# Amanda-Zheng/MR-GNAS

Hardware: AMD Instinct MI355X
Metric: million edges/sec per supernet fwd+bwd step (FB15k-237, dim=200) (higher is better)
Workload: dtype f32

## Files before the change

### mr-gnas_amd/csrc/wgrad.hip

```cpp
#include "x3_parts.hpp"
#include "wgrad_plan.hpp"

static_assert(mrg::WGRAD_BLOCK == MRG_BLOCK, "wgrad_plan.hpp plans for workgroups of MRG_BLOCK threads");

namespace mrg {

struct WgradArgs {
  const float* gY; int Nout; int ldg;
  const float* X1; const float* X2; int K1, K2;
  float* ws;
  int64_t rows, rows_per_block;
  int TM, TN, TNB;
  int ngrp;
  int64_t g_lo[3], g_hi[3], g_rpb[3], g_ws_off[3];
  int g_G[3];
};

struct XSel { const float* base; int ld, kk; };
__device__ __forceinline__ XSel wgrad_sel_x(const WgradArgs& a, int c) {
  const bool first = c < a.K1 || a.K2 == 0;
  XSel s;
  s.base = first ? a.X1 : a.X2;
  s.ld = first ? a.K1 : a.K2;
  s.kk = first ? c : c - a.K1;
// ... 391 lines not shown
  const int tn0 = (int)(((int64_t)blockIdx.y * a.TN) / gridDim.y);
  const int tnb = (int)(((int64_t)(blockIdx.y + 1) * a.TN) / gridDim.y) - tn0;
  const int tid = threadIdx.x, wave = __builtin_amdgcn_readfirstlane(tid >> 6), lane = tid & 63, li = lane & 31, lh = lane >> 5;
  const int wg = wave / KP, wp = wave % KP;
  const int m0 = wg * 4;
  const int an = a.TM - m0 < 4 ? (a.TM - m0 > 0 ? a.TM - m0 : 0) : 4;
  const int kn = tnb - 2 * wp < 2 ? (tnb - 2 * wp > 0 ? tnb - 2 * wp : 0) : 2;
  const int K = a.K1 + a.K2;

  f32x16 acc[4][2];
#pragma unroll
  for (int i = 0; i < 4; ++i)
#pragma unroll
    for (int j = 0; j < 2; ++j)
#pragma unroll
      for (int r = 0; r < 16; ++r) acc[i][j][r] = 0.f;

  int64_t r_begin = (int64_t)blockIdx.x * a.rows_per_block;
  int64_t r_end = r_begin + a.rows_per_block;
  if (r_end > a.rows) r_end = a.rows;
  int64_t ws_off = 0;
  if (a.ngrp > 0) {
    const int z = blockIdx.z;
#define MRG_PICKZ(F) (z == 0 ? a.F[0] : (z == 1 ? a.F[1] : a.F[2]))
    if ((int)blockIdx.x >= MRG_PICKZ(g_G)) return;
    const int64_t rpb = MRG_PICKZ(g_rpb), hi = MRG_PICKZ(g_hi);
    r_begin = MRG_PICKZ(g_lo) + (int64_t)blockIdx.x * rpb;
    r_end = r_begin + rpb < hi ? r_begin + rpb : hi;
    ws_off = MRG_PICKZ(g_ws_off);
#undef MRG_PICKZ
  }

  const float* src[FPW]; int64_t ld[FPW]; bool live[FPW];
#pragma unroll
  for (int i = 0; i < FPW; ++i) {
    const int f = wave + 8 * i;
    live[i] = f < NFRAG && (f < ASLOTS ? f < a.TM : f - ASLOTS < tnb);
    const float* base = mrg_zeros16; int64_t l = 0;
    if (live[i]) {
      if (f < ASLOTS) {
        const int cg = f * 32 + li;
        if (cg < a.Nout) { base = a.gY + (r_begin + 8 * lh) * a.ldg + cg; l = a.ldg; }
      } else {
        const int cg = (tn0 + f - ASLOTS) * 32 + li;
        if (cg < K) {
          const XSel sx = wgrad_sel_x(a, cg);
          base = sx.base + (r_begin + 8 * lh) * sx.ld + sx.kk; l = sx.ld;
        } else if (cg == K) {
          base = mrg_ones16;
        }
      }
    }
    src[i] = base; ld[i] = l;
  }
  constexpr unsigned BUF_BYTES = X::BUF_BYTES;

  const int64_t nfull = (r_end - r_begin) / WBR;
  const int nv_tail = (int)((r_end - r_begin) - nfull * WBR);
  const int kbase = 8 * lh;
  float raw[FPW][8];
  auto fetch = [&](int64_t t) {
    const int64_t toff = t * WBR;
#pragma unroll
    for (int i = 0; i < FPW; ++i) {
      const float* p = src[i] + toff * ld[i];
#pragma unroll
      for (int j = 0; j < 8; ++j) raw[i][j] = p[j * ld[i]];
    }
  };
  auto produce = [&](int buf, auto tail_c) {
    constexpr bool TAIL = decltype(tail_c)::value;
#pragma unroll
    for (int i = 0; i < FPW; ++i) {
      if (live[i]) {
        float x[8];
#pragma unroll
        for (int j = 0; j < 8; ++j) x[j] = (!TAIL || kbase + j < nv_tail) ? raw[i][j] : 0.f;
        u32x4 H, M, L;
        split8(x, H, M, L);
        const int f = wave + 8 * i;
        u32x4* dst = reinterpret_cast<u32x4*>(reinterpret_cast<char*>(smem) + buf * BUF_BYTES + f * X::FRAG_BYTES) + lane;
        dst[0] = H; dst[64] = M; dst[128] = L;
      }
    }
  };
  auto rdfrag = [&](int buf, int f, bf16x8& H, bf16x8& M, bf16x8& L) {
    const u32x4* p = reinterpret_cast<const u32x4*>(reinterpret_cast<const char*>(smem) + buf * BUF_BYTES + f * X::FRAG_BYTES) + lane;
    H = __builtin_bit_cast(bf16x8, p[0]); M = __builtin_bit_cast(bf16x8, p[64]); L = __builtin_bit_cast(bf16x8, p[128]);
  };
  auto consume = [&](int cur) {
    if (an > 0 && kn > 0) {
      bf16x8 Bh0, Bm0, Bl0, Bh1, Bm1, Bl1;
      rdfrag(cur, ASLOTS + 2 * wp, Bh0, Bm0, Bl0);
      if (kn > 1) rdfrag(cur, ASLOTS + 2 * wp + 1, Bh1, Bm1, Bl1);
      else { Bh1 = Bh0; Bm1 = Bm0; Bl1 = Bl0; }
      bf16x8 An[3];
      rdfrag(cur, m0, An[0], An[1], An[2]);
#pragma unroll
      for (int i = 0; i < 4; ++i) {
        if (i < an) {
          const bf16x8 Ah = An[0], Am = An[1], Al = An[2];
          if (i + 1 < an) rdfrag(cur, m0 + i + 1, An[0], An[1], An[2]);
          if (kn > 1) {
            x3_chain2(acc[i][0], acc[i][1], Ah, Am, Al, Bh0, Bm0, Bl0, Ah, Am, Al, Bh1, Bm1, Bl1);
          } else {
            x3_chain(acc[i][0], Ah, Am, Al, Bh0, Bm0, Bl0);
          }
        }
      }
    }
  };

  if (nfull > 0) {
    fetch(0);
    produce(0, std::false_type{});
    fetch(nfull > 1 ? 1 : 0);
    __syncthreads();
    int cur = 0;
    for (int64_t t = 0; t < nfull; ++t) {
      consume(cur);
      if (t + 1 < nfull) produce(cur ^ 1, std::false_type{});
      fetch(t + 2 < nfull ? t + 2 : nfull - 1);
      __syncthreads();
      cur ^= 1;
    }
  }
  if (nv_tail > 0) {
    const int64_t toff = nfull * WBR;
#pragma unroll
    for (int i = 0; i < FPW; ++i) {
      const float* p = src[i] + toff * ld[i];
#pragma unroll
      for (int j = 0; j < 8; ++j) raw[i][j] = p[(int64_t)(kbase + j >= nv_tail ? j - WBR : j) * ld[i]];
    }
    produce(0, std::true_type{});
    __syncthreads();
    consume(0);
  }
  const int ldw = a.TN * 32;
  float* out = a.ws + ws_off + (int64_t)blockIdx.x * (a.TM * 32) * ldw;
#pragma unroll
  for (int i = 0; i < 4; ++i)
#pragma unroll
    for (int j = 0; j < 2; ++j)
      if (i < an && j < kn) {
#pragma unroll
        for (int r = 0; r < 16; ++r) {
          const int row = (m0 + i) * 32 + (r & 3) + 8 * (r >> 2) + 4 * lh;
          out[(int64_t)row * ldw + (tn0 + 2 * wp + j) * 32 + li] = acc[i][j][r];
        }
      }
}

static int launch_wgrad_x3(const WgradArgs& a, int G, int nrange, hipStream_t st) {
  bool v1 = gemm_switches().wgrad_variant == 1 && a.rows >= WBR;
  for (int i = 0; i < a.ngrp; ++i) v1 = v1 && !(a.g_hi[i] > a.g_lo[i] && a.g_hi[i] < WBR);
  auto go = [&](auto ng_c) {
    using X = WgradX3<decltype(ng_c)::value>;
    const dim3 grid(G, (a.TN + X::KT - 1) / X::KT, nrange);
    if (v1) return launch_kernel(wgrad_x3v_k<decltype(ng_c)::value>, grid, dim3(WX_THREADS), X::LDS_SPLIT, st, a);
    return launch_kernel(wgrad_x3_k<decltype(ng_c)::value>, grid, dim3(WX_THREADS), X::LDS_RAW, st, a);
  };
  return a.TM <= 4 ? go(std::integral_constant<int, 1>{}) : go(std::integral_constant<int, 2>{});
}

struct WgradReduce3 { const float* ws[3]; float* gW[3]; float* gbias[3]; int G[3]; };
__global__ void wgrad_reduce3_k(WgradReduce3 p, int K, int Nout, int ldg, int ldx) {
  __shared__ float part[16][64];
  const int z = blockIdx.z;
  const float* __restrict__ ws = z == 0 ? p.ws[0] : (z == 1 ? p.ws[1] : p.ws[2]);
  float* __restrict__ gW = z == 0 ? p.gW[0] : (z == 1 ? p.gW[1] : p.gW[2]);
  float* __restrict__ gbias = z == 0 ? p.gbias[0] : (z == 1 ? p.gbias[1] : p.gbias[2]);
  const int G = z == 0 ? p.G[0] : (z == 1 ? p.G[1] : p.G[2]);
  if (!gW) return;
  const int tx = threadIdx.x & 63, ty = threadIdx.x >> 6;
  const int c = blockIdx.x * 64 + tx;
  const int n = blockIdx.y;
  float acc = 0.f;
  if (c <= K)
    for (int g = ty; g < G; g += 16) acc += ws[((int64_t)g * ldg + n) * ldx + c];
  part[ty][tx] = acc;
  __syncthreads();
  if (ty == 0 && c <= K) {
    float tot = part[0][tx];
#pragma unroll
    for (int i = 1; i < 16; ++i) tot += part[i][tx];
    if (c < K) gW[(int64_t)n * K + c] = tot;
    else if (gbias) gbias[n] = tot;
  }
}

static int launch_wgrad_reduce(const WgradReduce3& red, int nrange, int K, int Nout, int TM, int TN, hipStream_t st) {
  hipLaunchKernelGGL(wgrad_reduce3_k, dim3((K + 1 + 63) / 64, Nout, nrange), dim3(1024), 0, st, red, K, Nout, TM * 32, TN * 32);
  MRG_LAUNCH_CHECK();
  return MRG_OK;
}

static int64_t wgrad_workspace_bytes(int64_t rows, int K, int Nout) {
  WgradPlan p = wgrad_plan(rows, K, Nout);
  return (int64_t)p.G * p.TM * 32 * p.TN * 32 * sizeof(float);
}

static bool wgrad_vec_ok(const float* gY, int ldg, const float* X1, const float* X2, int K1, int K2, int Nout) {
  const bool shape = Nout >= 4 && Nout % 4 == 0 && ldg % 4 == 0 && K1 >= 4 && K1 % 4 == 0 && K2 >= 0 && K2 % 4 == 0;
  return shape && aligned16(gY) && aligned16(X1) && (!X2 || K2 == 0 || aligned16(X2));
}

static int launch_wgrad_one(const float* gY, int ldg, const float* X1, const float* X2, int K1, int K2, float* gW, float* gbias, void* ws,
                            int64_t rows, int Nout, int share, hipStream_t st) {
  const int K = K1 + K2;
  if (rows == 0) {
    hipError_t e = hipMemsetAsync(gW, 0, sizeof(float) * (size_t)Nout * K, st);
    if (e == hipSuccess && gbias) e = hipMemsetAsync(gbias, 0, sizeof(float) * (size_t)Nout, st);
    return (int)e;
  }
  const bool vec = Nout <= 224 && wgrad_vec_ok(gY, ldg, X1, X2, K1, K2, Nout);
  WgradPlan p = wgrad_plan(rows, K, Nout, vec, share);
  if (!p.ok) return MRG_E_SHAPE;
  WgradArgs a{};
  a.gY = gY; a.Nout = Nout; a.ldg = ldg; a.X1 = X1; a.X2 = X2; a.K1 = K1; a.K2 = K2; a.ws = (float*)ws;
  a.rows = rows; a.rows_per_block = p.rows_per_block; a.TM = p.TM; a.TN = p.TN; a.TNB = p.TNB;
  if (!X2 || K2 == 0) { a.X2 = X1; a.K2 = 0; }
  int rc = MRG_E_SHAPE;
  if (vec && gemm_switches().mode != 1) {
    rc = launch_wgrad_x3(a, p.G, 1, st);
  } else {
    const dim3 grid(p.G, (p.TN + p.TNB - 1) / p.TNB);
    const int npf = wgrad_npf_class(p.npf);
    void (*kernel)(WgradArgs) = nullptr;
#define MRG_WGRAD_DMA(T, F) if (vec && p.tpw == T && npf == F) kernel = wgrad_dma_k<T, F>;
#define MRG_WGRAD_PLAIN(T, F) if (!vec && p.tpw == T && npf == F) kernel = wgrad_k<T, F>;
    MRG_WGRAD_DMA_INSTANCES(MRG_WGRAD_DMA) MRG_WGRAD_PLAIN_INSTANCES(MRG_WGRAD_PLAIN)
#undef MRG_WGRAD_DMA
#undef MRG_WGRAD_PLAIN
    if (kernel) rc = launch_kernel(kernel, grid, dim3(MRG_BLOCK), p.lds, st, a);
  }
  if (rc != MRG_OK) return rc;
  const WgradReduce3 red{{(const float*)ws}, {gW}, {gbias}, {p.G}};
  return launch_wgrad_reduce(red, 1, K, Nout, p.TM, p.TN, st);
}

struct Wgrad3Layout { int64_t lo[3], hi[3], off[3], total; WgradPlan plan[3]; };
static Wgrad3Layout wgrad3_layout(int64_t b0, int64_t b1, int64_t M, int K, int Nout, int share) {
  Wgrad3Layout L{{0, b0, b1}, {b0, b1, M}};
  for (int i = 0; i < 3; ++i) {
    L.plan[i] = wgrad_plan(L.hi[i] - L.lo[i], K, Nout, true, share);
    L.off[i] = L.total;
    L.total += (wgrad_workspace_bytes(L.hi[i] - L.lo[i], K, Nout) + 255) / 256 * 256;
  }
  return L;
}

}

using namespace mrg;

extern "C" int mrg_wgrad_set_variant(int variant) {
  if (variant != 0 && variant != 1) return MRG_E_ENUM;
  gemm_switches().wgrad_variant = variant;
  return MRG_OK;
}

extern "C" int64_t mrg_linear_bwd_weight3_workspace_bytes(int64_t b0, int64_t b1, int64_t M, int K1, int K2, int Nout) {
  if (M < 0 || b0 < 0 || b1 < b0 || M < b1 || Nout > 224 || !wgrad_vec_ok(nullptr, Nout, nullptr, nullptr, K1, K2, Nout) || gemm_switches().mode == 1) return 0;
  return wgrad3_layout(b0, b1, M, K1 + K2, Nout, 1).total;
}

extern "C" int mrg_linear_bwd_weight3(const float* gY, const float* X1, const float* X2, float* const* gW_host, float* const* gb_host, void* ws,
                                      int64_t b0, int64_t b1, int64_t M, int K1, int K2, int Nout, void* stream) {
  if (M < 0 || b0 < 0 || b1 < b0 || M < b1 || Nout > 224 || !wgrad_vec_ok(nullptr, Nout, nullptr, nullptr, K1, K2, Nout)) return MRG_E_SHAPE;
  if (!gW_host) return MRG_E_NULLPTR;
  if (M > 0 && (!gY || !X1 || (K2 > 0 && !X2))) return MRG_E_NULLPTR;
  if (!ws) return MRG_E_WORKSPACE;
  if (!wgrad_vec_ok(gY, Nout, X1, X2, K1, K2, Nout)) return MRG_E_SHAPE;
  const int K = K1 + K2;
  const int64_t rows[3] = {b0, b1 - b0, M - b1};
  int nlive = 0;
  for (int i = 0; i < 3; ++i) nlive += (gW_host[i] != nullptr && rows[i] > 0) ? 1 : 0;
  const Wgrad3Layout L = wgrad3_layout(b0, b1, M, K, Nout, nlive < 1 ? 1 : nlive);
  if (!L.plan[0].ok) return MRG_E_SHAPE;
  WgradArgs a{};
  a.gY = gY; a.Nout = Nout; a.ldg = Nout; a.X1 = X1; a.X2 = K2 > 0 ? X2 : X1; a.K1 = K1; a.K2 = K2; a.ws = (float*)ws; a.rows = M;
  a.TM = L.plan[0].TM; a.TN = L.plan[0].TN; a.TNB = L.plan[0].TNB; a.ngrp = 3;
  WgradReduce3 red{};
  int maxG = 0;
  for (int i = 0; i < 3; ++i) {
    const WgradPlan& p = L.plan[i];
    const bool live = gW_host[i] != nullptr;
    a.g_lo[i] = L.lo[i]; a.g_hi[i] = L.hi[i]; a.g_rpb[i] = p.rows_per_block; a.g_G[i] = live ? p.G : 0; a.g_ws_off[i] = L.off[i] / (int64_t)sizeof(float);
    red.ws[i] = (const float*)((const char*)ws + L.off[i]); red.gW[i] = gW_host[i]; red.gbias[i] = gb_host ? gb_host[i] : nullptr; red.G[i] = p.G;
    if (live && p.G > maxG) maxG = p.G;
  }
  if (maxG == 0) return MRG_OK;
  const int rc = launch_wgrad_x3(a, maxG, 3, (hipStream_t)stream);
  return rc != MRG_OK ? rc : launch_wgrad_reduce(red, 3, K, Nout, a.TM, a.TN, (hipStream_t)stream);
}

extern "C" int64_t mrg_linear_bwd_weight_workspace_bytes(int64_t rows, int K, int Nout) {
  if (rows < 0 || K <= 0 || Nout <= 0) return 0;
  return wgrad_workspace_bytes(rows, K, Nout);
}

extern "C" int mrg_linear_bwd_weight_share(const float* gY, const float* X1, const float* X2, float* gW, float* gbias, void* ws,
                                           int64_t rows, int K1, int K2, int Nout, int share, void* stream) {
  if (rows < 0 || K1 <= 0 || K2 < 0 || Nout <= 0) return MRG_E_SHAPE;
  if (share < 1 || share > 3) return MRG_E_ENUM;
  if (!gW) return MRG_E_NULLPTR;
  if (rows > 0 && (!gY || !X1 || (K2 > 0 && !X2))) return MRG_E_NULLPTR;
  if (rows > 0 && !ws) return MRG_E_WORKSPACE;
  if (K2 == 0) X2 = nullptr;
  int cw = Nout;
  if (Nout > 224 && rows > 0 && wgrad_vec_ok(gY, Nout, X1, X2, K1, K2, Nout)) {
    const int nblk = (Nout + 223) / 224;
    cw = (((Nout + nblk - 1) / nblk) + 31) / 32 * 32;
  }
  for (int n0 = 0; n0 < Nout; n0 += cw) {
    const int nc = Nout - n0 < cw ? Nout - n0 : cw;
    int rc = launch_wgrad_one(gY + n0, Nout, X1, X2, K1, K2, gW + (int64_t)n0 * (K1 + K2), gbias ? gbias + n0 : nullptr, ws, rows, nc, share, (hipStream_t)stream);
    if (rc != MRG_OK) return rc;
  }
  return MRG_OK;
}

extern "C" int mrg_linear_bwd_weight(const float* gY, const float* X1, const float* X2, float* gW, float* gbias, void* ws,
                                     int64_t rows, int K1, int K2, int Nout, void* stream) {
  return mrg_linear_bwd_weight_share(gY, X1, X2, gW, gbias, ws, rows, K1, K2, Nout, 1, stream);
}
```

### mr-gnas_amd/csrc/wgrad_plan.hpp

```cpp
#pragma once
#include <stddef.h>
#include <stdint.h>

namespace mrg {

constexpr int WBR = 16;
constexpr int WGRAD_BLOCK = 256;

struct WgradPlan {
  int TM, TN, TNB, tpw, npf, G;
  int64_t rows_per_block;
  size_t lds;
  bool ok;
};

constexpr int WGRAD_SHARE_MAX_BLOCKS = 400;

inline WgradPlan wgrad_plan(int64_t rows, int K, int Nout, bool dma = false, int share = 1) {
  WgradPlan p{};
  p.TM = (Nout + 31) / 32;
  p.TN = (K + 1 + 31) / 32;
  const int opts[] = {1, 2, 4, 7};
  if (dma && p.TM <= 7) {
    p.TNB = p.TN < 4 ? p.TN : 4;
    for (int o : opts) if (p.TM <= o) { p.tpw = o; break; }
  } else {
    p.TNB = p.TM * p.TN <= 28 ? p.TN : (28 / p.TM > 0 ? 28 / p.TM : 0);
    int per_wave = p.TNB > 0 ? (p.TM * p.TNB + 3) / 4 : 99;
    for (int o : opts) if (per_wave <= o) { p.tpw = o; break; }
  }
  int nf4 = WBR * (p.TM + p.TNB) * 8;
  p.npf = (nf4 + WGRAD_BLOCK - 1) / WGRAD_BLOCK;
  p.lds = (size_t)(dma ? 3 : 2) * WBR * (p.TM + p.TNB) * 32 * sizeof(float);
  p.ok = p.tpw > 0 && p.lds <= 160 * 1024 && p.npf <= 16;
  int64_t tiles = (rows + WBR - 1) / WBR;
  const int ny = (p.TN + (p.TM <= 4 ? 16 : 8) - 1) / (p.TM <= 4 ? 16 : 8);
  const bool shared = share > 1 && (tiles + 15) / 16 <= WGRAD_SHARE_MAX_BLOCKS;
  const int64_t gshare = 256 / (ny * share);
  const int64_t gmax = !shared ? (256 / ny > 32 ? 256 / ny : 32) : (gshare > 16 ? gshare : 16);
  int64_t G = (tiles + 15) / 16 < gmax ? (tiles + 15) / 16 : gmax;
  const int64_t gsmall = (tiles + 3) / 4 < 8 ? (tiles + 3) / 4 : 8;
  if (G < gsmall) G = gsmall;
  if (G < 1) G = 1;
  int64_t tpb = (tiles + G - 1) / G;
  if (tpb < 1) tpb = 1;
  p.rows_per_block = tpb * WBR;
  p.G = (int)((rows + p.rows_per_block - 1) / p.rows_per_block);
  if (p.G < 1) p.G = 1;
  return p;
}

inline int wgrad_npf_class(int npf) { return npf <= 2 ? 2 : (npf <= 4 ? 4 : (npf <= 8 ? 8 : 16)); }

#define MRG_WGRAD_DMA_INSTANCES(X) X(1, 2) X(1, 4) X(2, 2) X(2, 4) X(4, 2) X(4, 4) X(7, 4) X(7, 8)
#define MRG_WGRAD_PLAIN_INSTANCES(X) X(1, 2) X(1, 4) X(2, 4) X(2, 8) X(4, 4) X(4, 8) X(4, 16) X(7, 8) X(7, 16)

inline bool wgrad_has_instance(bool dma, int tpw, int npf_class) {
#define MRG_WGRAD_IS(T, F) if (tpw == T && npf_class == F) return true;
  if (dma) { MRG_WGRAD_DMA_INSTANCES(MRG_WGRAD_IS) } else { MRG_WGRAD_PLAIN_INSTANCES(MRG_WGRAD_IS) }
#undef MRG_WGRAD_IS
  return false;
}

}
```

### mr-gnas_amd/csrc/x3_parts.hpp

```cpp
#pragma once
#include <type_traits>
#include "gemm.hpp"

namespace mrg {

typedef __bf16 bf16x8 __attribute__((ext_vector_type(8)));
typedef __bf16 bf16x2 __attribute__((ext_vector_type(2)));
typedef float f32x2 __attribute__((ext_vector_type(2)));
typedef float f32x4v __attribute__((ext_vector_type(4)));
typedef unsigned u32x4 __attribute__((ext_vector_type(4)));

constexpr int64_t X3N_MAX_ROWS = 16384;
struct GemmSwitches {
  int mode = 0;
  int q = 1;
  int64_t small_rows = X3N_MAX_ROWS;
  int wide8 = 1;
  int wgrad_variant = 1;
};
inline GemmSwitches& gemm_switches() { static GemmSwitches s; return s; }

__device__ __forceinline__ float sub1(float a, float b) {
  float r;
  asm("v_sub_f32 %0, %1, %2" : "=v"(r) : "v"(a), "v"(b));
  return r;
}
__device__ __forceinline__ void split_pair(float x0, float x1, unsigned& h, unsigned& m, unsigned& l) {
  f32x2 v = {x0, x1};
  h = __builtin_bit_cast(unsigned, __builtin_convertvector(v, bf16x2));
  f32x2 r = {sub1(x0, __builtin_bit_cast(float, h << 16)), sub1(x1, __builtin_bit_cast(float, h & 0xffff0000u))};
  m = __builtin_bit_cast(unsigned, __builtin_convertvector(r, bf16x2));
  f32x2 r2 = {sub1(r.x, __builtin_bit_cast(float, m << 16)), sub1(r.y, __builtin_bit_cast(float, m & 0xffff0000u))};
  l = __builtin_bit_cast(unsigned, __builtin_convertvector(r2, bf16x2));
}
__device__ __forceinline__ void split8(const float (&v)[8], u32x4& H, u32x4& M, u32x4& L) {
#pragma unroll
  for (int j = 0; j < 4; ++j) {
    unsigned h, m, l;
    split_pair(v[2 * j], v[2 * j + 1], h, m, l);
    H[j] = h; M[j] = m; L[j] = l;
  }
}
__device__ __forceinline__ void split_pair_of(const v4f (&x)[2], int q, u32x4& H, u32x4& M, u32x4& L) {
  const v4f& v = x[q >> 1];
  unsigned h, m, l;
  if (q & 1) split_pair(v.z, v.w, h, m, l); else split_pair(v.x, v.y, h, m, l);
  H[q] = h; M[q] = m; L[q] = l;
}

__device__ __forceinline__ f32x16 x3_mm(bf16x8 a, bf16x8 b, f32x16 c) { return __builtin_amdgcn_mfma_f32_32x32x16_bf16(a, b, c, 0, 0, 0); }
__device__ __forceinline__ f32x4v x3_mm(bf16x8 a, bf16x8 b, f32x4v c) { return __builtin_amdgcn_mfma_f32_16x16x32_bf16(a, b, c, 0, 0, 0); }
template <class ACC>
__device__ __forceinline__ void x3_chain(ACC& c, bf16x8 Ah, bf16x8 Am, bf16x8 Al, bf16x8 Bh, bf16x8 Bm, bf16x8 Bl) {
  c = x3_mm(Am, Bm, c);
  c = x3_mm(Al, Bh, c);
  c = x3_mm(Ah, Bl, c);
  c = x3_mm(Am, Bh, c);
  c = x3_mm(Ah, Bm, c);
  c = x3_mm(Ah, Bh, c);
}
__device__ __forceinline__ void x3_chain2(f32x16& c0, f32x16& c1, bf16x8 Ah0, bf16x8 Am0, bf16x8 Al0, bf16x8 Bh0, bf16x8 Bm0, bf16x8 Bl0,
                                          bf16x8 Ah1, bf16x8 Am1, bf16x8 Al1, bf16x8 Bh1, bf16x8 Bm1, bf16x8 Bl1) {
  c0 = x3_mm(Am0, Bm0, c0); c1 = x3_mm(Am1, Bm1, c1);
  c0 = x3_mm(Al0, Bh0, c0); c1 = x3_mm(Al1, Bh1, c1);
  c0 = x3_mm(Ah0, Bl0, c0); c1 = x3_mm(Ah1, Bl1, c1);
  c0 = x3_mm(Am0, Bh0, c0); c1 = x3_mm(Am1, Bh1, c1);
  c0 = x3_mm(Ah0, Bm0, c0); c1 = x3_mm(Ah1, Bm1, c1);
  c0 = x3_mm(Ah0, Bh0, c0); c1 = x3_mm(Ah1, Bh1, c1);
}
template <int MT, int NT>
__device__ __forceinline__ void x3_chain_rows(f32x16 (&acc)[MT][NT], int n, const u32x4 (&Ah)[MT], const u32x4 (&Am)[MT], const u32x4 (&Al)[MT],
                                              bf16x8 Bh, bf16x8 Bm, bf16x8 Bl) {
  static_assert(MT == 1 || MT == 2, "one or two row tiles per wave");
  auto c = [](const u32x4& v) { return __builtin_bit_cast(bf16x8, v); };
  if constexpr (MT == 2) x3_chain2(acc[0][n], acc[1][n], c(Ah[0]), c(Am[0]), c(Al[0]), Bh, Bm, Bl, c(Ah[1]), c(Am[1]), c(Al[1]), Bh, Bm, Bl);
  else x3_chain(acc[0][n], c(Ah[0]), c(Am[0]), c(Al[0]), Bh, Bm, Bl);
}

inline int x3_tiles(int N, int nt) { return ((N + nt * 32 - 1) / (nt * 32)) * nt; }
inline int x3_slabs(int K) { return (K + 15) / 16; }
inline size_t x3_bsplit_bytes(int N, int K, int nt) { return (size_t)x3_slabs(K) * x3_tiles(N, nt) * 3 * 64 * 16; }
struct BSplitTiles32 {
  static __host__ __device__ int chunks(int ntile, int nslab) { return nslab * ntile * 64; }
  static __host__ __device__ int tiles(int ntile, int) { return ntile; }
  static __device__ __forceinline__ void source(int lane, int tile, int slab, int& n, int& k0) {
    n = tile * 32 + (lane & 31); k0 = slab * 16 + (lane >> 5) * 8;
  }
};
constexpr int X3Q_HT = 7;
constexpr int X3Q_NT = 2 * X3Q_HT;
struct BSplitTiles16 {
  static __host__ __device__ int chunks(int nslab) { return nslab * X3Q_NT * 64; }
  static __host__ __device__ int tiles(int) { return X3Q_NT; }
  static __device__ __forceinline__ void source(int lane, int tile, int slab, int& n, int& k0) {
    n = tile * 16 + (lane & 15); k0 = slab * 32 + (lane >> 4) * 8;
  }
};
struct BSplit3 { const float* B[3]; u32x4* out[3]; const float* B2[3]; int ksplit; };
template <class LAYOUT, class... DIMS>
static __global__ void bsplit_k(BSplit3 p, int64_t sn, int64_t sk, int N, int K, DIMS... dims) {
  const float* __restrict__ B = p.B[blockIdx.y];
  const float* __restrict__ B2 = p.B2[blockIdx.y];
  const int ksplit = (p.ksplit > 0 && B2) ? p.ksplit : K;
  u32x4* __restrict__ Bp = p.out[blockIdx.y];
  if (!B) return;
  const int idx = blockIdx.x * blockDim.x + threadIdx.x;
  if (idx >= LAYOUT::chunks(dims...)) return;
  const int ntile = LAYOUT::tiles(dims...);
  const int lane = idx & 63, tile = (idx >> 6) % ntile, slab = (idx >> 6) / ntile;
  int n, k0;
  LAYOUT::source(lane, tile, slab, n, k0);
  float v[8];
#pragma unroll
  for (int j = 0; j < 8; ++j) {
    const int k = k0 + j;
    v[j] = (n < N && k < K) ? (k < ksplit ? B[n * sn + k * sk] : B2[n * sn + (k - ksplit) * sk]) : 0.f;
  }
  u32x4 h, m, l;
#pragma unroll
  for (int j = 0; j < 4; ++j) {
    unsigned a, b, c;
    split_pair(v[2 * j], v[2 * j + 1], a, b, c);
    h[j] = a; m[j] = b; l[j] = c;
  }
  u32x4* o = Bp + ((int64_t)(slab * ntile + tile) * 3) * 64 + lane;
  o[0] = h; o[64] = m; o[128] = l;
}
template <class LAYOUT, class... DIMS>
inline void launch_bsplit_layout(const float* const* B, int64_t sn, int64_t sk, int N, int K, void* const* out, int count, hipStream_t st,
                                 const float* const* B2, int ksplit, DIMS... dims) {
  BSplit3 p{};
  for (int i = 0; i < count; ++i) { p.B[i] = B[i]; p.out[i] = (u32x4*)out[i]; p.B2[i] = B2 ? B2[i] : nullptr; }
  p.ksplit = B2 ? ksplit : 0;
  hipLaunchKernelGGL((bsplit_k<LAYOUT, DIMS...>), dim3((LAYOUT::chunks(dims...) + 255) / 256, count), dim3(256), 0, st, p, sn, sk, N, K, dims...);
}
inline void launch_bsplit3(const float* const* B, int64_t sn, int64_t sk, int N, int K, int nt, void* const* out, hipStream_t st,
                           const float* const* B2 = nullptr, int ksplit = 0) {
  const int ntile = x3_tiles(N, nt), nslab = x3_slabs(K);
  launch_bsplit_layout<BSplitTiles32>(B, sn, sk, N, K, out, 3, st, B2, ksplit, ntile, nslab);
}
inline void launch_bsplit(const float* B, int64_t sn, int64_t sk, int N, int K, int nt, void* Bp, hipStream_t st) {
  const int ntile = x3_tiles(N, nt), nslab = x3_slabs(K);
  launch_bsplit_layout<BSplitTiles32>(&B, sn, sk, N, K, &Bp, 1, st, nullptr, 0, ntile, nslab);
}
inline int x3q_slabs(int K) { return (K + 31) / 32; }
inline void launch_bsplitq3(const float* const* B, int64_t sn, int64_t sk, int N, int K, void* const* out, int count, hipStream_t st,
                            const float* const* B2 = nullptr, int ksplit = 0) {
  const int nslab = x3q_slabs(K);
  launch_bsplit_layout<BSplitTiles16>(B, sn, sk, N, K, out, count, st, B2, ksplit, nslab);
}

__device__ __forceinline__ void wait_vmcnt(int n) {
#define MRG_VM(N) case N: asm volatile("s_waitcnt vmcnt(" #N ")" ::: "memory"); break;
  switch (n) {
    MRG_VM(0) MRG_VM(1) MRG_VM(2) MRG_VM(3) MRG_VM(4) MRG_VM(5) MRG_VM(6) MRG_VM(7)
    MRG_VM(8) MRG_VM(9) MRG_VM(10) MRG_VM(11) MRG_VM(12) MRG_VM(13) MRG_VM(14) MRG_VM(15)
    MRG_VM(16) MRG_VM(17) MRG_VM(18) MRG_VM(19) MRG_VM(20) MRG_VM(21) MRG_VM(22) MRG_VM(23)
    MRG_VM(24) MRG_VM(25) MRG_VM(26) MRG_VM(27) MRG_VM(28) MRG_VM(29) MRG_VM(30) MRG_VM(31)
    MRG_VM(32) MRG_VM(33) MRG_VM(34) MRG_VM(35) MRG_VM(36) MRG_VM(37) MRG_VM(38) MRG_VM(39)
    MRG_VM(40) MRG_VM(41) MRG_VM(42) MRG_VM(43) MRG_VM(44) MRG_VM(45) MRG_VM(46) MRG_VM(47)
    MRG_VM(48) MRG_VM(49) MRG_VM(50) MRG_VM(51) MRG_VM(52) MRG_VM(53) MRG_VM(54) MRG_VM(55)
    MRG_VM(56) MRG_VM(57) MRG_VM(58) MRG_VM(59) MRG_VM(60) MRG_VM(61) MRG_VM(62)
    default: asm volatile("s_waitcnt vmcnt(63)" ::: "memory"); break;
  }
#undef MRG_VM
}

#define MRG_PICK(F) (sg == 0 ? a.grp.F[0] : (sg == 1 ? a.grp.F[1] : a.grp.F[2]))
#define MRG_GROUP_SELECT(GBM)                                                                                          \
  int64_t row0 = (int64_t)blockIdx.x * (GBM);                                                                          \
  int sg = 0;                                                                                                          \
// ... 53 lines not shown
```

Baseline: 11.95.

## Add 16x16-tile wave-mapped wgrad kernel with hold/stream fragment reuse

Adds a new weight-gradient kernel that splits the output into 16x16 tiles and assigns each of 8 waves a rectangle of tiles chosen by a host-side load-balancing planner. Each wave holds up to 4 fragments and streams up to 7 against them, using the bf16x3 split MFMA chain and double-buffered LDS with register prefetch. Row-per-block counts are rounded to even tiles. It becomes the default via wgrad_variant=2 for Nout in (128,208], aiming to raise MFMA utilization and cut LDS reads for the dim=200 shapes, at the cost of a large LDS footprint and one block per CU.

```diff
diff --git a/mr-gnas_amd/csrc/wgrad.hip b/mr-gnas_amd/csrc/wgrad.hip
--- a/mr-gnas_amd/csrc/wgrad.hip
+++ b/mr-gnas_amd/csrc/wgrad.hip
@@ -567,8 +567,15 @@
       }
 }
 
-static int launch_wgrad_x3(const WgradArgs& a, int G, int nrange, hipStream_t st) {
-  bool v1 = gemm_switches().wgrad_variant == 1 && a.rows >= WBR;
+}
+
+#include "wgrad_w.hpp"
+
+namespace mrg {
+
+static int launch_wgrad_x3(const WgradArgs& a, int G, int nrange, hipStream_t st, bool w) {
+  if (w) return launch_wgrad_w(a, G, nrange, st);
+  bool v1 = gemm_switches().wgrad_variant >= 1 && a.rows >= WBR;
   for (int i = 0; i < a.ngrp; ++i) v1 = v1 && !(a.g_hi[i] > a.g_lo[i] && a.g_hi[i] < WBR);
   auto go = [&](auto ng_c) {
     using X = WgradX3<decltype(ng_c)::value>;
@@ -630,7 +637,8 @@
     return (int)e;
   }
   const bool vec = Nout <= 224 && wgrad_vec_ok(gY, ldg, X1, X2, K1, K2, Nout);
-  WgradPlan p = wgrad_plan(rows, K, Nout, vec, share);
+  const bool w = gemm_switches().mode != 1 && wgrad_w_takes(gemm_switches().wgrad_variant, vec, rows, K, Nout, share);
+  WgradPlan p = wgrad_plan(rows, K, Nout, vec, share, w);
   if (!p.ok) return MRG_E_SHAPE;
   WgradArgs a{};
   a.gY = gY; a.Nout = Nout; a.ldg = ldg; a.X1 = X1; a.X2 = X2; a.K1 = K1; a.K2 = K2; a.ws = (float*)ws;
@@ -638,7 +646,7 @@
   if (!X2 || K2 == 0) { a.X2 = X1; a.K2 = 0; }
   int rc = MRG_E_SHAPE;
   if (vec && gemm_switches().mode != 1) {
-    rc = launch_wgrad_x3(a, p.G, 1, st);
+    rc = launch_wgrad_x3(a, p.G, 1, st, w);
   } else {
     const dim3 grid(p.G, (p.TN + p.TNB - 1) / p.TNB);
     const int npf = wgrad_npf_class(p.npf);
@@ -656,10 +664,10 @@
 }
 
 struct Wgrad3Layout { int64_t lo[3], hi[3], off[3], total; WgradPlan plan[3]; };
-static Wgrad3Layout wgrad3_layout(int64_t b0, int64_t b1, int64_t M, int K, int Nout, int share) {
+static Wgrad3Layout wgrad3_layout(int64_t b0, int64_t b1, int64_t M, int K, int Nout, int share, bool w = false) {
   Wgrad3Layout L{{0, b0, b1}, {b0, b1, M}};
   for (int i = 0; i < 3; ++i) {
-    L.plan[i] = wgrad_plan(L.hi[i] - L.lo[i], K, Nout, true, share);
+    L.plan[i] = wgrad_plan(L.hi[i] - L.lo[i], K, Nout, true, share, w);
     L.off[i] = L.total;
     L.total += (wgrad_workspace_bytes(L.hi[i] - L.lo[i], K, Nout) + 255) / 256 * 256;
   }
@@ -671,7 +679,7 @@
 using namespace mrg;
 
 extern "C" int mrg_wgrad_set_variant(int variant) {
-  if (variant != 0 && variant != 1) return MRG_E_ENUM;
+  if (variant < 0 || variant > 2) return MRG_E_ENUM;
   gemm_switches().wgrad_variant = variant;
   return MRG_OK;
 }
@@ -692,7 +700,9 @@
   const int64_t rows[3] = {b0, b1 - b0, M - b1};
   int nlive = 0;
   for (int i = 0; i < 3; ++i) nlive += (gW_host[i] != nullptr && rows[i] > 0) ? 1 : 0;
-  const Wgrad3Layout L = wgrad3_layout(b0, b1, M, K, Nout, nlive < 1 ? 1 : nlive);
+  const int share = nlive < 1 ? 1 : nlive;
+  const bool w = gemm_switches().mode != 1 && wgrad_w_takes3(gemm_switches().wgrad_variant, b0, b1, M, K, Nout, share);
+  const Wgrad3Layout L = wgrad3_layout(b0, b1, M, K, Nout, share, w);
   if (!L.plan[0].ok) return MRG_E_SHAPE;
   WgradArgs a{};
   a.gY = gY; a.Nout = Nout; a.ldg = Nout; a.X1 = X1; a.X2 = K2 > 0 ? X2 : X1; a.K1 = K1; a.K2 = K2; a.ws = (float*)ws; a.rows = M;
@@ -707,7 +717,7 @@
     if (live && p.G > maxG) maxG = p.G;
   }
   if (maxG == 0) return MRG_OK;
-  const int rc = launch_wgrad_x3(a, maxG, 3, (hipStream_t)stream);
+  const int rc = launch_wgrad_x3(a, maxG, 3, (hipStream_t)stream, w);
   return rc != MRG_OK ? rc : launch_wgrad_reduce(red, 3, K, Nout, a.TM, a.TN, (hipStream_t)stream);
 }
 
diff --git a/mr-gnas_amd/csrc/wgrad_plan.hpp b/mr-gnas_amd/csrc/wgrad_plan.hpp
--- a/mr-gnas_amd/csrc/wgrad_plan.hpp
+++ b/mr-gnas_amd/csrc/wgrad_plan.hpp
@@ -16,7 +16,7 @@
 
 constexpr int WGRAD_SHARE_MAX_BLOCKS = 400;
 
-inline WgradPlan wgrad_plan(int64_t rows, int K, int Nout, bool dma = false, int share = 1) {
+inline WgradPlan wgrad_plan(int64_t rows, int K, int Nout, bool dma = false, int share = 1, bool even = false) {
   WgradPlan p{};
   p.TM = (Nout + 31) / 32;
   p.TN = (K + 1 + 31) / 32;
@@ -44,6 +44,7 @@
   if (G < 1) G = 1;
   int64_t tpb = (tiles + G - 1) / G;
   if (tpb < 1) tpb = 1;
+  if (even) tpb += tpb & 1;
   p.rows_per_block = tpb * WBR;
   p.G = (int)((rows + p.rows_per_block - 1) / p.rows_per_block);
   if (p.G < 1) p.G = 1;
diff --git a/mr-gnas_amd/csrc/wgrad_w.hpp b/mr-gnas_amd/csrc/wgrad_w.hpp
--- /dev/null
+++ b/mr-gnas_amd/csrc/wgrad_w.hpp
@@ -0,0 +1,227 @@
+#pragma once
+#include "wgrad_w_map.hpp"
+
+namespace mrg {
+
+static_assert(WGRAD_W_MIN_ROWS >= WW_ROWS, "the ragged period reads the 32 rows that end at the range's end");
+constexpr int WW_THREADS = 512;
+constexpr int WW_FRAG_BYTES = 3 * 1024;
+constexpr unsigned WW_BUF_BYTES = 2 * WW_MAXT * WW_FRAG_BYTES;
+constexpr size_t WW_LDS = (size_t)2 * WW_BUF_BYTES;
+struct WwArgs { unsigned map[2][WW_WAVES]; int TA, TQ; };
+
+__global__ __launch_bounds__(WW_THREADS, 1) void wgrad_x3w_k(WgradArgs a, WwArgs m) {
+  extern __shared__ __align__(16) float smem[];
+  char* const lds = reinterpret_cast<char*>(smem);
+  const int ny = gridDim.y;
+  const int tn0 = (int)(((int64_t)blockIdx.y * m.TQ) / ny);
+  const int tnb = (int)(((int64_t)(blockIdx.y + 1) * m.TQ) / ny) - tn0;
+  const int tid = threadIdx.x, wave = __builtin_amdgcn_readfirstlane(tid >> 6), lane = tid & 63, li = lane & 31, lh = lane >> 5;
+  const int K = a.K1 + a.K2;
+
+#define MRG_WW_PICK(M) (wave == 0 ? M[0] : wave == 1 ? M[1] : wave == 2 ? M[2] : wave == 3 ? M[3] : wave == 4 ? M[4] : wave == 5 ? M[5] : wave == 6 ? M[6] : M[7])
+  const bool wide = tnb * ny >= m.TQ;
+  const unsigned rect = __builtin_amdgcn_readfirstlane(wide ? MRG_WW_PICK(m.map[0]) : MRG_WW_PICK(m.map[1]));
+#undef MRG_WW_PICK
+  const int ra0 = rect & 15, ran = (rect >> 4) & 15, rb0 = (rect >> 8) & 15, rbn = (rect >> 12) & 15;
+  const bool hold_a = (rect >> 16) & 1;
+  const int hn = hold_a ? ran : rbn, sn = hold_a ? rbn : ran;
+  const int hf = hold_a ? ra0 : WW_MAXT + rb0, sf = hold_a ? WW_MAXT + rb0 : ra0;
+
+  int64_t r_begin = (int64_t)blockIdx.x * a.rows_per_block;
+  int64_t r_end = r_begin + a.rows_per_block;
+  if (r_end > a.rows) r_end = a.rows;
+  int64_t ws_off = 0;
+  if (a.ngrp > 0) {
+    const int z = blockIdx.z;
+#define MRG_PICKZ(F) (z == 0 ? a.F[0] : (z == 1 ? a.F[1] : a.F[2]))
+    if ((int)blockIdx.x >= MRG_PICKZ(g_G)) return;
+    const int64_t rpb = MRG_PICKZ(g_rpb), hi = MRG_PICKZ(g_hi);
+    r_begin = MRG_PICKZ(g_lo) + (int64_t)blockIdx.x * rpb;
+    r_end = r_begin + rpb < hi ? r_begin + rpb : hi;
+    ws_off = MRG_PICKZ(g_ws_off);
+#undef MRG_PICKZ
+  }
+
+  const int nA = (m.TA + 1) >> 1;
+  const int bc0 = tn0 * 16, bc1 = bc0 + tnb * 16;
+  const int e1 = bc1 < a.K1 ? bc1 : a.K1;
+  const int n1 = e1 > bc0 ? (e1 - bc0 + 31) >> 5 : 0;
+  const int s2 = bc0 > a.K1 ? bc0 : a.K1, e2 = bc1 < K ? bc1 : K;
+  const int w2 = (s2 - bc0) >> 5;
+  const int n2 = e2 > s2 ? ((e2 - bc0 + 31) >> 5) - w2 : 0;
+  const float* ub[2]; int64_t uld[2]; unsigned voff[2]; int fb[2]; bool live[2], act[2];
+#pragma unroll
+  for (int i = 0; i < 2; ++i) {
+    const int u = wave + 8 * i;
+    ub[i] = a.gY; uld[i] = 0; voff[i] = 0; fb[i] = 0; live[i] = false; act[i] = false;
+    if (u < nA) {
+      const int col = 32 * u + li;
+      live[i] = true; act[i] = col < a.Nout;
+      ub[i] = a.gY + r_begin * a.ldg; uld[i] = a.ldg;
+      voff[i] = (unsigned)(8 * lh * a.ldg + (act[i] ? col : a.Nout - 1)) * 4u;
+      fb[i] = 2 * u;
+    } else if (u - nA < n1) {
+      const int w = u - nA, cg = bc0 + 32 * w + li;
+      live[i] = true; act[i] = cg < e1;
+      ub[i] = a.X1 + r_begin * a.K1; uld[i] = a.K1;
+      voff[i] = (unsigned)(8 * lh * a.K1 + (act[i] ? cg : e1 - 1)) * 4u;
+      fb[i] = WW_MAXT + 2 * w;
+    } else if (u - nA - n1 < n2) {
+      const int w = w2 + (u - nA - n1), cg = bc0 + 32 * w + li;
+      live[i] = true; act[i] = cg >= s2 && cg < e2;
+      ub[i] = a.X2 + r_begin * a.K2; uld[i] = a.K2;
+      voff[i] = (unsigned)(8 * lh * a.K2 + (cg < s2 ? s2 : (cg < e2 ? cg : e2 - 1)) - a.K1) * 4u;
+      fb[i] = WW_MAXT + 2 * w;
+    }
+  }
+  const unsigned dlane = (unsigned)((li >> 4) * WW_FRAG_BYTES + (lh * 16 + (li & 15)) * 16);
+
+#pragma unroll 1
+  for (unsigned c = tid; c < WW_LDS / 16; c += WW_THREADS) reinterpret_cast<u32x4*>(lds)[c] = u32x4{0u, 0u, 0u, 0u};
+  __syncthreads();
+  const bool has_ones = bc0 <= K && K < bc1;
+  const unsigned ones_off = (unsigned)((WW_MAXT + ((K - bc0) >> 4)) * WW_FRAG_BYTES + ((K - bc0) & 15) * 16);
+  if (has_ones && tid < 8)
+    *reinterpret_cast<u32x4*>(lds + (tid >> 2) * WW_BUF_BYTES + ones_off + (tid & 3) * 256) = u32x4{0x3F803F80u, 0x3F803F80u, 0x3F803F80u, 0x3F803F80u};
+
+  const int64_t nfull = (r_end - r_begin) / WW_ROWS;
+  const int nv_tail = (int)((r_end - r_begin) - nfull * WW_ROWS);
+  float raw[2][2][8];
+  auto fetch_unit = [&](int i, int64_t t) __attribute__((always_inline)) {
+    const float* tb = ub[i] + t * WW_ROWS * uld[i];
+#pragma unroll
+    for (int q = 0; q < 2; ++q)
+#pragma unroll
+      for (int j = 0; j < 8; ++j)
+        raw[i][q][j] = *reinterpret_cast<const float*>(reinterpret_cast<const char*>(tb + (16 * q + j) * uld[i]) + voff[i]);
+  };
+  auto fetch = [&](int64_t t) __attribute__((always_inline)) { fetch_unit(0, t); fetch_unit(1, t); };
+  auto produce = [&](int buf, int c, auto tail_c) __attribute__((always_inline)) {
+    constexpr bool TAIL = decltype(tail_c)::value;
+    const int i = c >> 1, q = c & 1;
+    if (live[i]) {
+      float x[8];
+#pragma unroll
+      for (int j = 0; j < 8; ++j) x[j] = (!TAIL || 16 * q + 8 * lh + j < nv_tail) ? raw[i][q][j] : 0.f;
+      u32x4 H, M, L;
+      split8(x, H, M, L);
+      if (act[i]) {
+        u32x4* d = reinterpret_cast<u32x4*>(lds + (buf * WW_BUF_BYTES + fb[i] * WW_FRAG_BYTES + q * 512) + dlane);
+        d[0] = H; d[64] = M; d[128] = L;
+      }
+    }
+  };
+  auto rdfrag = [&](int buf, int f, u32x4 (&P)[3]) __attribute__((always_inline)) {
+    const u32x4* p = reinterpret_cast<const u32x4*>(lds + buf * WW_BUF_BYTES + f * WW_FRAG_BYTES) + lane;
+    P[0] = p[0]; P[1] = p[64]; P[2] = p[128];
+  };
+  auto barrier = [&]() __attribute__((always_inline)) { asm volatile("s_waitcnt lgkmcnt(0)\n\ts_barrier" ::: "memory"); };
+  auto tail_produce = [&](int buf) __attribute__((always_inline)) {
+#pragma unroll
+    for (int i = 0; i < 2; ++i)
+#pragma unroll
+      for (int q = 0; q < 2; ++q) {
+#pragma unroll
+        for (int j = 0; j < 8; ++j) {
+          const int k = 16 * q + 8 * lh + j;
+          const float* tb = ub[i] + ((nfull - 1) * WW_ROWS + 16 * q + j) * uld[i];
+          const unsigned vo = voff[i] + (k >= nv_tail ? 0u : (unsigned)(WW_ROWS * 4) * (unsigned)uld[i]);
+          raw[i][q][j] = *reinterpret_cast<const float*>(reinterpret_cast<const char*>(tb) + vo);
+        }
+        __builtin_amdgcn_sched_barrier(0);
+      }
+#pragma unroll
+    for (int c = 0; c < 4; ++c) produce(buf, c, std::true_type{});
+    if (has_ones && tid < 4) {
+      u32x4 v;
+#pragma unroll
+      for (int p = 0; p < 4; ++p) v[p] = (8 * tid + 2 * p < nv_tail ? 0x3F80u : 0u) | (8 * tid + 2 * p + 1 < nv_tail ? 0x3F800000u : 0u);
+      *reinterpret_cast<u32x4*>(lds + buf * WW_BUF_BYTES + ones_off + tid * 256) = v;
+    }
+  };
+  const int64_t nper = nfull + (nv_tail > 0 ? 1 : 0);
+  const int ldw = a.TN * 32;
+  float* const out = a.ws + ws_off + (int64_t)blockIdx.x * (a.TM * 32) * ldw;
+
+  auto run = [&](auto hn_c, auto hold_c) __attribute__((always_inline)) {
+    constexpr int HN = decltype(hn_c)::value, HR = HN > 0 ? HN : 1, HPP = HN == 4 ? 1 : HR;
+    constexpr bool HA = decltype(hold_c)::value;
+    auto bf = [](const u32x4& v) { return __builtin_bit_cast(bf16x8, v); };
+    f32x4v acc[WW_STREAM][HR];
+#pragma unroll
+    for (int s = 0; s < WW_STREAM; ++s)
+#pragma unroll
+      for (int h = 0; h < HR; ++h)
+#pragma unroll
+        for (int r = 0; r < 4; ++r) acc[s][h][r] = 0.f;
+    if (nfull > 0) {
+      fetch(0);
+#pragma unroll
+      for (int c = 0; c < 4; ++c) produce(0, c, std::false_type{});
+      fetch(nfull > 1 ? 1 : 0);
+    } else if (nv_tail > 0) {
+      tail_produce(0);
+    }
+    barrier();
+    int cur = 0;
+#pragma unroll 1
+    for (int64_t t = 0; t < nper; ++t) {
+#pragma unroll
+      for (int p = 0; p < HN / HPP; ++p) {
+        u32x4 Hd[HPP][3];
+#pragma unroll
+        for (int h = 0; h < HPP; ++h) rdfrag(cur, hf + p * HPP + h, Hd[h]);
+#pragma unroll
+        for (int s = 0; s < WW_STREAM; ++s) {
+          if (s < sn) {
+            u32x4 S[3];
+            rdfrag(cur, sf + s, S);
+#pragma unroll
+            for (int h = 0; h < HPP; ++h) {
+              if (HA) x3_chain(acc[s][p * HPP + h], bf(Hd[h][0]), bf(Hd[h][1]), bf(Hd[h][2]), bf(S[0]), bf(S[1]), bf(S[2]));
+              else x3_chain(acc[s][p * HPP + h], bf(S[0]), bf(S[1]), bf(S[2]), bf(Hd[h][0]), bf(Hd[h][1]), bf(Hd[h][2]));
+            }
+            __builtin_amdgcn_sched_barrier(0);
+          }
+        }
+      }
+#pragma unroll
+      for (int c = 0; c < 4; ++c) produce(cur ^ 1, c, std::false_type{});
+      if (t + 1 == nfull && nv_tail > 0) tail_produce(cur ^ 1);
+      else if (nfull > 0) fetch(t + 2 < nfull ? t + 2 : nfull - 1);
+      barrier();
+      cur ^= 1;
+    }
+    const int lc = lane & 15, lg = lane >> 4;
+#pragma unroll
+    for (int s = 0; s < WW_STREAM; ++s)
+#pragma unroll
+      for (int h = 0; h < HN; ++h)
+        if (s < sn) {
+          const int ai = ra0 + (HA ? h : s), bj = rb0 + (HA ? s : h);
+#pragma unroll
+          for (int r = 0; r < 4; ++r) out[(int64_t)(ai * 16 + 4 * lg + r) * ldw + (tn0 + bj) * 16 + lc] = acc[s][h][r];
+        }
+  };
+#define MRG_WW_CASE(N) case N: if (hold_a) run(std::integral_constant<int, N>{}, std::true_type{}); else run(std::integral_constant<int, N>{}, std::false_type{}); break;
+  switch (hn) {
+    MRG_WW_CASE(1) MRG_WW_CASE(2) MRG_WW_CASE(3) MRG_WW_CASE(4)
+    default: run(std::integral_constant<int, 0>{}, std::false_type{}); break;
+  }
+#undef MRG_WW_CASE
+}
+
+
+static int launch_wgrad_w(const WgradArgs& a, int G, int nrange, hipStream_t st) {
+  WwArgs m{};
+  m.TA = wgrad_w_row_tiles(a.Nout);
+  m.TQ = wgrad_w_col_tiles(a.K1 + a.K2);
+  const int ny = wgrad_w_blocks(m.TQ);
+  const WwMap wide = wgrad_w_map(m.TA, (m.TQ + ny - 1) / ny), narrow = wgrad_w_map(m.TA, m.TQ / ny);
+  if (!wide.ok || !narrow.ok) return MRG_E_SHAPE;
+  for (int w = 0; w < WW_WAVES; ++w) { m.map[0][w] = wgrad_w_pack(wide.w[w]); m.map[1][w] = wgrad_w_pack(narrow.w[w]); }
+  return launch_kernel(wgrad_x3w_k, dim3(G, ny, nrange), dim3(WW_THREADS), WW_LDS, st, a, m);
+}
+
+}
diff --git a/mr-gnas_amd/csrc/wgrad_w_map.hpp b/mr-gnas_amd/csrc/wgrad_w_map.hpp
--- /dev/null
+++ b/mr-gnas_amd/csrc/wgrad_w_map.hpp
@@ -0,0 +1,99 @@
+#pragma once
+#include <stdint.h>
+
+namespace mrg {
+
+constexpr int WW_ROWS = 32;
+constexpr int WW_MAXT = 13;
+constexpr int WW_WAVES = 8;
+constexpr int WW_HOLD = 4;
+constexpr int WW_STREAM = 7;
+constexpr int64_t WGRAD_W_MIN_ROWS = 32;
+
+struct WwRect { int a0, an, b0, bn; bool hold_a; };
+struct WwMap { WwRect w[WW_WAVES]; int busiest; int reads; bool ok; };
+
+inline bool ww_rect_fits(int an, int bn, bool& hold_a) {
+  hold_a = false;
+  if (an == 0 || bn == 0) return true;
+  if (bn <= an) {
+    if (bn <= WW_HOLD && an <= WW_STREAM) return true;
+    if (an <= WW_HOLD && bn <= WW_STREAM) { hold_a = true; return true; }
+  } else {
+    if (an <= WW_HOLD && bn <= WW_STREAM) { hold_a = true; return true; }
+    if (bn <= WW_HOLD && an <= WW_STREAM) return true;
+  }
+  return false;
+}
+
+inline WwMap wgrad_w_map(int TA, int TB) {
+  WwMap best{};
+  best.busiest = 1 << 30;
+  if (TA < 1 || TB < 1 || TA > WW_MAXT || TB > WW_MAXT) return best;
+  for (int side = 0; side < 2; ++side) {
+    const int P = side == 0 ? TA : TB, S = side == 0 ? TB : TA;
+    const int g[2] = {(P + 1) / 2, P - (P + 1) / 2};
+    for (int n0 = 1; n0 <= WW_WAVES; ++n0) {
+      const int n[2] = {n0, WW_WAVES - n0};
+      if ((g[1] > 0) != (n[1] > 0)) continue;
+      WwRect r[WW_WAVES];
+      bool fits = true;
+      int reads = 0, k = 0;
+      for (int grp = 0; grp < 2; ++grp)
+        for (int i = 0; i < n[grp]; ++i, ++k) {
+          const int s0 = i * S / n[grp], sn = (i + 1) * S / n[grp] - s0;
+          const int p0 = grp == 0 ? 0 : g[0], pn = sn > 0 ? g[grp] : 0;
+          r[k] = side == 0 ? WwRect{p0, pn, s0, sn, false} : WwRect{s0, sn, p0, pn, false};
+          if (r[k].an == 0 || r[k].bn == 0) r[k] = WwRect{0, 0, 0, 0, false};
+          fits = fits && ww_rect_fits(r[k].an, r[k].bn, r[k].hold_a);
+          reads += r[k].an + r[k].bn;
+        }
+      if (!fits) continue;
+      int order[WW_WAVES];
+      for (int i = 0; i < WW_WAVES; ++i) order[i] = i;
+      for (int i = 1; i < WW_WAVES; ++i)
+        for (int j = i; j > 0 && r[order[j]].an * r[order[j]].bn > r[order[j - 1]].an * r[order[j - 1]].bn; --j) {
+          const int t = order[j]; order[j] = order[j - 1]; order[j - 1] = t;
+        }
+      WwMap m{};
+      for (int s = 0; s < 4; ++s) {
+        m.w[s] = r[order[s]];
+        m.w[s + 4] = r[order[WW_WAVES - 1 - s]];
+        const int load = m.w[s].an * m.w[s].bn + m.w[s + 4].an * m.w[s + 4].bn;
+        if (load > m.busiest) m.busiest = load;
+      }
+      m.reads = reads;
+      if (m.busiest < best.busiest || (m.busiest == best.busiest && m.reads < best.reads)) best = m;
+    }
+  }
+  best.ok = best.busiest < (1 << 30) && best.busiest * 169 <= 46 * TA * TB;
+  return best;
+}
+
+inline int wgrad_w_row_tiles(int Nout) { return (Nout + 15) / 16; }
+inline int wgrad_w_col_tiles(int K) { return (K + 1 + 15) / 16; }
+inline int wgrad_w_blocks(int TQ) { return (TQ + WW_MAXT - 1) / WW_MAXT; }
+
+inline bool wgrad_w_shape(int K, int Nout) {
+  if (Nout <= 128 || Nout > 16 * WW_MAXT || K < 1) return false;
+  const int TA = wgrad_w_row_tiles(Nout), TQ = wgrad_w_col_tiles(K), ny = wgrad_w_blocks(TQ);
+  const int wide = (TQ + ny - 1) / ny, narrow = TQ / ny;
+  return wgrad_w_map(TA, wide).ok && (narrow == wide || wgrad_w_map(TA, narrow).ok);
+}
+
+inline bool wgrad_w_takes(int variant, bool vec, int64_t rows, int K, int Nout, int share) {
+  (void)share;
+  return variant == 2 && vec && rows >= WGRAD_W_MIN_ROWS && wgrad_w_shape(K, Nout);
+}
+inline bool wgrad_w_takes3(int variant, int64_t b0, int64_t b1, int64_t M, int K, int Nout, int share) {
+  const int64_t rows[3] = {b0, b1 - b0, M - b1};
+  for (int i = 0; i < 3; ++i)
+    if (rows[i] > 0 && rows[i] < WW_ROWS) return false;
+  return wgrad_w_takes(variant, true, M, K, Nout, share);
+}
+
+inline uint32_t wgrad_w_pack(const WwRect& r) {
+  return (uint32_t)r.a0 | (uint32_t)r.an << 4 | (uint32_t)r.b0 << 8 | (uint32_t)r.bn << 12 | (r.hold_a ? 1u << 16 : 0u);
+}
+
+}
diff --git a/mr-gnas_amd/csrc/x3_parts.hpp b/mr-gnas_amd/csrc/x3_parts.hpp
--- a/mr-gnas_amd/csrc/x3_parts.hpp
+++ b/mr-gnas_amd/csrc/x3_parts.hpp
@@ -16,7 +16,7 @@
   int q = 1;
   int64_t small_rows = X3N_MAX_ROWS;
   int wide8 = 1;
-  int wgrad_variant = 1;
+  int wgrad_variant = 2;
 };
 inline GemmSwitches& gemm_switches() { static GemmSwitches s; return s; }
 
```

Result: no change. 11.99, median of 4 (+0.3%).
